# maximyudayev/Realtime-ST-GCN

Hardware: AMD Instinct MI355X
Metric: skeleton-frames/sec/GPU (fwd+bwd), 10-layer ST-GCN N=64 T=300 V=25 (higher is better)
Workload: dtype bf16; 1 GPU; config 2: as_is st-gcn (fcn_in + 9 StgcnLayer, BatchNorm, Kt=9), fwd + loss + bwd + Adam; global_batch=64, seq_len=300, joints=25, parallelism=single, bn_stats=per-replica, launch=eager

## Files before the change

realtime-st-gcn_amd/csrc/wgrad_wide.hip:

```cpp
#include "common.h"
#include "launchers.h"
#include "lds_ops.h"
#include "../../include/stgcn_amd.h"
#include <stdlib.h>

namespace {

constexpr int NT = 512;
constexpr int KM = 128;
constexpr int PR = 64;
constexpr int COB = 128, CIB = 64;
constexpr int DY_PANEL = KM * PR;
constexpr int DY_BYTES = (COB / 32) * DY_PANEL;
constexpr int DY_U = KM * (COB / 8) / NT;
constexpr int X_U = (KM * (CIB / 8) + NT - 1) / NT;
constexpr int LDS_MAX = 160 * 1024;

struct WWGeom {
  int F;
  int RS;
  int MS;
  int nco, nci;
  int tiles_n;
  int tpb;
  int R;
  int fold;
  int cin_f;
  float* slab;
};

template <int PRO, int KTAP>
__global__ __launch_bounds__(NT, 1) void wgrad_wide_kernel(const stgcn_wgrad_desc a, const WWGeom g) {
  constexpr int KT = KTAP, PADT = (KTAP - 1) / 2;
  extern __shared__ __attribute__((aligned(16))) char smem[];
  const int V = a.V, F = g.F;
  const int XP = g.MS * V * PR;
  char* const sX = smem;
  char* const sY = smem + 2 * XP;
  const int tid = threadIdx.x, lane = tid & 63, wave = tid >> 6;
  const int wc = wave >> 1, wi = wave & 1;
  {
    uint4* z = reinterpret_cast<uint4*>(smem);
    const int nz = (2 * XP + 2 * DY_BYTES) / 16;
    for (int e = tid; e < nz; e += NT) z[e] = make_uint4(0, 0, 0, 0);
    __syncthreads();
  }
  const int ob = blockIdx.x % (g.nco * g.nci), rg = blockIdx.x / (g.nco * g.nci);
  const int co0 = (ob % g.nco) * COB, cf0 = (ob / g.nco) * CIB;
  const int par = g.fold ? cf0 / a.Cin : 0;
  const int ci0 = cf0 - par * a.Cin;
  const int fmul = g.fold ? 2 : 1;
  const int tiles_n = g.tiles_n;
  const int k_begin = rg * g.tpb, k_end = min(a.N * tiles_n, k_begin + g.tpb);

  const bf16* __restrict__ xin = reinterpret_cast<const bf16*>(a.in);
  const bf16* __restrict__ dy = reinterpret_cast<const bf16*>(a.dy);

  const int ycu = tid & 15, xcu = tid & 7;
  float sc[8], sh[8];
  if (PRO == 1) {
#pragma unroll
    for (int j = 0; j < 8; ++j) {
      const int c = ci0 + xcu * 8 + j;
      sc[j] = c < a.Cin ? a.pro_a[c] : 0.f;
      sh[j] = c < a.Cin ? a.pro_b[c] : 0.f;
    }
  }
  constexpr bool AHEAD2 = KT < 9;
  uint4 ry[2][DY_U], rx[2][X_U];
  const bool ycok = co0 + ycu * 8 < a.Cout, xcok = ci0 + xcu * 8 < a.Cin;
  const bf16* __restrict__ dyb = dy + co0 + (ycok ? ycu * 8 : 0);
  const bf16* __restrict__ xb = xin + ci0 + (xcok ? xcu * 8 : 0);
  auto load_dy = [&]<int S>(int n, int f0) {
    f0 = min(f0, a.T_out - 1);
    const int rows_valid = min(F, a.T_out - f0) * V;
    const bf16* base = dyb + ((long)n * a.T_out + f0) * V * a.dy_ld;
    static_for<DY_U>([&]<int i>() {
      const int r = (tid >> 4) + 32 * i;
      ry[S][i] = *reinterpret_cast<const uint4*>(base + (long)(r < rows_valid ? r : 0) * a.dy_ld);
    });
  };
  auto store_dy = [&]<int S>(int buf, int f0) {
    const int rows_valid = ycok ? min(F, a.T_out - f0) * V : 0;
    char* p = sY + buf * DY_BYTES + (ycu >> 2) * DY_PANEL + (ycu & 3) * 16;
    static_for<DY_U>([&]<int i>() {
      const int r = (tid >> 4) + 32 * i;
      *reinterpret_cast<uint4*>(p + r * PR) = r < rows_valid ? ry[S][i] : make_uint4(0, 0, 0, 0);
    });
  };
  auto load_x = [&]<int S>(int n, int fa, int nf) {
    static_for<X_U>([&]<int i>() {
      const int r = (tid >> 3) + 64 * i;
      const int rr = r < nf * V ? r : 0;
      const int fl = rr / V, v = rr - fl * V, f = fa + fl;
      const int fs = min(max(fmul * f + par, 0), a.T_in - 1);
      rx[S][i] = *reinterpret_cast<const uint4*>(xb + (((long)n * a.T_in + fs) * V + v) * a.in_ld);
    });
  };
  auto store_x = [&]<int S>(int fa, int nf) {
    static_for<X_U>([&]<int i>() {
      const int r = (tid >> 3) + 64 * i;
      if (r < nf * V) {
        const int fl = r / V, v = r - fl * V, f = fa + fl;
        const bool ok = xcok && f >= 0 && fmul * f + par < a.T_in;
        uint4 u = ok ? rx[S][i] : make_uint4(0, 0, 0, 0);
        if (PRO == 1 && ok) {
          float e[8];
          unpack16(u, e, (bf16*)nullptr);
#pragma unroll
          for (int j = 0; j < 8; ++j) e[j] = fmaxf(fmaf(e[j], sc[j], sh[j]), 0.f);
          u = pack16(e, (bf16*)nullptr);
        }
        int slot = f % g.RS;
        slot += slot < 0 ? g.RS : 0;
        char* p = sX + (xcu >> 2) * XP + (xcu & 3) * 16 + v * PR;
        *reinterpret_cast<uint4*>(p + slot * V * PR) = u;
        if (slot + g.RS < g.MS) *reinterpret_cast<uint4*>(p + (slot + g.RS) * V * PR) = u;
      }
    });
  };
  auto stage_window = [&]<int S>(int n, int f0) {
    for (int fb = f0 - PADT; fb < f0 + F + PADT; fb += F) {
      const int nf = min(F, f0 + F + PADT - fb);
      load_x.template operator()<S>(n, fb, nf);
      store_x.template operator()<S>(fb, nf);
    }
  };

  const int li = lane & 15, gq = lane >> 4;
  const int colb = (16 * (gq & 1) + 4 * (li & 3)) * 2;
  const int rlo = 8 * (gq >> 1) + (li >> 2);

  f32x16 acc[KT];
#pragma unroll
  for (int t = 0; t < KT; ++t)
#pragma unroll
    for (int r = 0; r < 16; ++r) acc[t][r] = 0.f;

  for (int o = tid * 16; o < 2 * XP; o += NT * 16) *reinterpret_cast<uint4*>(sX + o) = make_uint4(0, 0, 0, 0);
  __syncthreads();

  const int tapb = V * PR;
  const int nk = k_end - k_begin;
  auto tile = [&]<int S>(int j) {
    const int k = k_begin + j;
    const int n = k / tiles_n, tt = k - n * tiles_n, f0 = tt * F;
    const bool next1 = j + 1 < nk && tt + 1 < tiles_n;
    if (tt == 0 || j == 0) {
      __syncthreads();
      load_dy.template operator()<S>(n, f0);
      store_dy.template operator()<S>(k & 1, f0);
      stage_window.template operator()<S>(n, f0);
      __syncthreads();
      if constexpr (AHEAD2) {
        load_dy.template operator()<S ^ 1>(n, f0 + F);
        load_x.template operator()<S ^ 1>(n, f0 + F + PADT, F);
      }
    }
    if constexpr (AHEAD2) {
      load_dy.template operator()<S>(n, f0 + 2 * F);
      load_x.template operator()<S>(n, f0 + 2 * F + PADT, F);
    } else {
      load_dy.template operator()<S ^ 1>(n, f0 + F);
      load_x.template operator()<S ^ 1>(n, f0 + F + PADT, F);
    }
    int s0 = (f0 - PADT) % g.RS;
    s0 += s0 < 0 ? g.RS : 0;
    const char* Y = sY + (k & 1) * DY_BYTES + wc * DY_PANEL + colb + rlo * PR;
    const char* X = sX + wi * XP + colb + (s0 * V + rlo) * PR;
    int tb = tapb;
    asm volatile("" : "+s"(tb));
    constexpr int NU = (KM / 16) * KT, D = 2;
    bf16x8 fx[D + 1], fy[2];
    auto rd = [&]<int u>() {
      constexpr int ks = u / KT, t = u % KT;
      if constexpr (t == 0) fy[ks & 1] = trpair<PR>(Y + 16 * ks * PR);
      fx[u % (D + 1)] = trpair<PR>(X + t * tb + 16 * ks * PR);
    };
    static_for<D>([&]<int u>() { rd.template operator()<u>(); });
    static_for<NU>([&]<int u>() {
      if constexpr (u + D < NU) rd.template operator()<u + D>();
      constexpr int ks = u / KT, t = u % KT;
      acc[t] = __builtin_amdgcn_mfma_f32_32x32x16_bf16(fy[ks & 1], fx[u % (D + 1)], acc[t], 0, 0, 0);
    });
    if (next1) {
      store_dy.template operator()<S ^ 1>((k + 1) & 1, f0 + F);
      store_x.template operator()<S ^ 1>(f0 + F + PADT, F);
    }
    lds_barrier();
  };
  for (int j = 0; j < nk; j += 2) {
    tile.template operator()<0>(j);
    if (j + 1 < nk) tile.template operator()<1>(j + 1);
  }

  float* __restrict__ out = g.slab + (long)rg * KT * a.Cout * g.cin_f;
  const int ci = cf0 + 32 * wi + (lane & 31);
#pragma unroll
  for (int t = 0; t < KT; ++t)
#pragma unroll
    for (int r = 0; r < 16; ++r) {
      const int co = co0 + 32 * wc + acc_row(r, lane);
      if (co < a.Cout && ci < g.cin_f) out[((long)t * a.Cout + co) * g.cin_f + ci] = acc[t][r];
    }
}

struct WPlan {
  bool ok;
  WWGeom g;
  int ktap;
  size_t lds;
  long slab_elems;
};

constexpr int RS_PART = 16;

__global__ void unfold_reduce2_kernel(const float* __restrict__ part, int RS, int Cout, int Cin, float* __restrict__ dw,
                                      int mode) {
  const long E4 = 5L * Cout * 2 * Cin / 4;
  const long e4 = (long)blockIdx.x * blockDim.x + threadIdx.x;
  if (e4 >= E4) return;
  const long e = e4 * 4;
  const int cf = (int)(e % (2 * Cin));
  const long tc = e / (2 * Cin);
  const int co = (int)(tc % Cout), t = (int)(tc / Cout);
  const int par = cf / Cin, ci = cf - par * Cin, dt = 2 * t + par;
  if (dt > 8) return;
  float4 acc = make_float4(0.f, 0.f, 0.f, 0.f);
  for (int r = 0; r < RS; ++r) {
    const float4 v = *reinterpret_cast<const float4*>(part + (long)r * 4 * E4 + e);
    acc.x += v.x; acc.y += v.y; acc.z += v.z; acc.w += v.w;
  }
  if (mode) {
    float* d = dw + ((long)co * Cin + ci) * 9 + dt;
    d[0] = acc.x;
    d[9] = acc.y;
    d[18] = acc.z;
    d[27] = acc.w;
    return;
  }
  float4* d = reinterpret_cast<float4*>(dw + ((long)dt * Cout + co) * Cin + ci);
  float4 o = *d;
  o.x += acc.x; o.y += acc.y; o.z += acc.z; o.w += acc.w;
  *d = o;
}

WPlan wplan(const stgcn_wgrad_desc& a) {
  WPlan p{};
  p.ok = false;
  if (a.Kt != 9 || a.pad != 4) return p;
  WWGeom& g = p.g;
  if (a.stride == 1 && a.T_in == a.T_out) {
    g.fold = 0;
    p.ktap = 9;
    g.cin_f = a.Cin;
  } else if (a.stride == 2 && a.T_out == (a.T_in - 1) / 2 + 1 && a.Cin % CIB == 0) {
    g.fold = 1;
    p.ktap = 5;
    g.cin_f = 2 * a.Cin;
  } else {
    return p;
  }
  if (a.pro != 0 && a.pro != 1) return p;
  if (a.Cout < COB || a.Cin < CIB || a.Cout % 8 || a.Cin % 8 || a.in_ld % 8 || a.dy_ld % 8 || a.V > 32) return p;
  const int padt = (p.ktap - 1) / 2;
  g.F = KM / a.V;
  g.RS = 2 * g.F + 2 * padt;
  g.MS = g.RS + g.F + 2 * padt - 1;
  if (g.F < 1 || g.F * a.V > KM || g.F * a.V > 64 * X_U) return p;
  g.nco = (a.Cout + COB - 1) / COB;
  g.nci = (g.cin_f + CIB - 1) / CIB;
  const int nob = g.nco * g.nci;
  g.tiles_n = (a.T_out + g.F - 1) / g.F;
  const long total = (long)a.N * g.tiles_n;
  if (total > 0x7fffffffL) return p;
  int R = 256 / nob;
  if (R < 1) R = 1;
  if (R > total) R = (int)total;
  g.tpb = (int)((total + R - 1) / R);
  g.R = (int)((total + g.tpb - 1) / g.tpb);
  p.lds = 2 * (size_t)g.MS * a.V * PR + 2 * (size_t)DY_BYTES;
  if (p.lds > LDS_MAX || (size_t)(KM - g.F * a.V) * PR > 2 * (size_t)DY_BYTES) return p;
  p.slab_elems = (long)(g.R + RS_PART) * p.ktap * a.Cout * g.cin_f;
  p.ok = true;
  return p;
}

}

int slab_reduce_launch(const float* slab, int R, long E, float* part, float* dw, hipStream_t s, int mode, int Kt,
                       long CoCi);
int slab_reduce1_launch(const float* slab, int R, long E, float* part, hipStream_t s);

long wgrad_wide_workspace(const stgcn_wgrad_desc& a, int dtype) {
  if (dtype != 1) return 0;
  const WPlan p = wplan(a);
  return p.ok ? p.slab_elems * (long)sizeof(float) : 0;
}

int wgrad_wide_launch(const stgcn_wgrad_desc& a, int dtype, hipStream_t s) {
  if (dtype != 1 || a.work == nullptr) return -1;
  WPlan p = wplan(a);
  if (!p.ok || a.work_bytes < p.slab_elems * (long)sizeof(float)) return -1;
  p.g.slab = reinterpret_cast<float*>(a.work);
  auto* k = p.ktap == 9 ? (a.pro == 1 ? wgrad_wide_kernel<1, 9> : wgrad_wide_kernel<0, 9>)
                        : (a.pro == 1 ? wgrad_wide_kernel<1, 5> : wgrad_wide_kernel<0, 5>);
  if (stgcn_lds_attr((const void*)k, LDS_MAX, s)) return STGCN_EHIP;
  const unsigned grid = (unsigned)(p.g.nco * p.g.nci * p.g.R);
  hipLaunchKernelGGL(k, dim3(grid), dim3(NT), p.lds, s, a, p.g);
  if (hipGetLastError() != hipSuccess) return STGCN_EHIP;
  const long E = (long)p.ktap * a.Cout * p.g.cin_f;
  float* part = p.g.slab + (long)p.g.R * E;
  if (!p.g.fold) return slab_reduce_launch(p.g.slab, p.g.R, E, part, a.dw, s, a.out_mode, 9, (long)a.Cout * a.Cin);
  const int RS = slab_reduce1_launch(p.g.slab, p.g.R, E, part, s);
  if (RS < 0) return -RS;
  hipLaunchKernelGGL(unfold_reduce2_kernel, dim3((unsigned)((E / 4 + 255) / 256)), dim3(256), 0, s, (const float*)part,
                     RS, a.Cout, a.Cin, a.dw, a.out_mode);
  return hipGetLastError() == hipSuccess ? STGCN_OK : STGCN_EHIP;
}
```

Baseline: 2.573 million skeleton-frames/s.

## Skip structurally-zero last tap in folded wgrad and batch window loads

For the folded stride-2 case with KT=5 and odd parity, the kernel now instantiates a 4-tap MFMA loop and skips the final tap, whose weight-gradient slice is presumed structurally zero, so it does no work and no writeback for it. Window staging now issues all global loads for the three frame blocks into separate register buffers before any LDS stores, which exposes more memory-level parallelism. The redundant second LDS zeroing pass and one barrier are removed, and uniform values are hinted to scalar registers. The cost is higher register pressure and a duplicated code path; the unwritten slab entries must be zero or ignored downstream for the result to stay correct.

```diff
diff --git a/realtime-st-gcn_amd/csrc/wgrad_wide.hip b/realtime-st-gcn_amd/csrc/wgrad_wide.hip
--- a/realtime-st-gcn_amd/csrc/wgrad_wide.hip
+++ b/realtime-st-gcn_amd/csrc/wgrad_wide.hip
@@ -47,7 +47,7 @@
   }
   const int ob = blockIdx.x % (g.nco * g.nci), rg = blockIdx.x / (g.nco * g.nci);
   const int co0 = (ob % g.nco) * COB, cf0 = (ob / g.nco) * CIB;
-  const int par = g.fold ? cf0 / a.Cin : 0;
+  const int par = g.fold ? __builtin_amdgcn_readfirstlane(cf0 / a.Cin) : 0;
   const int ci0 = cf0 - par * a.Cin;
   const int fmul = g.fold ? 2 : 1;
   const int tiles_n = g.tiles_n;
@@ -67,7 +67,8 @@
     }
   }
   constexpr bool AHEAD2 = KT < 9;
-  uint4 ry[2][DY_U], rx[2][X_U];
+  constexpr int NB = 3;
+  uint4 ry[2][DY_U], rx[2 + NB][X_U];
   const bool ycok = co0 + ycu * 8 < a.Cout, xcok = ci0 + xcu * 8 < a.Cin;
   const bf16* __restrict__ dyb = dy + co0 + (ycok ? ycu * 8 : 0);
   const bf16* __restrict__ xb = xin + ci0 + (xcok ? xcu * 8 : 0);
@@ -88,7 +89,7 @@
       *reinterpret_cast<uint4*>(p + r * PR) = r < rows_valid ? ry[S][i] : make_uint4(0, 0, 0, 0);
     });
   };
-  auto load_x = [&]<int S>(int n, int fa, int nf) {
+  auto load_x = [&]<int S>(int n, int fa, int nf) __attribute__((always_inline)) {
     static_for<X_U>([&]<int i>() {
       const int r = (tid >> 3) + 64 * i;
       const int rr = r < nf * V ? r : 0;
@@ -97,7 +98,7 @@
       rx[S][i] = *reinterpret_cast<const uint4*>(xb + (((long)n * a.T_in + fs) * V + v) * a.in_ld);
     });
   };
-  auto store_x = [&]<int S>(int fa, int nf) {
+  auto store_x = [&]<int S>(int fa, int nf) __attribute__((always_inline)) {
     static_for<X_U>([&]<int i>() {
       const int r = (tid >> 3) + 64 * i;
       if (r < nf * V) {
@@ -119,12 +120,11 @@
       }
     });
   };
-  auto stage_window = [&]<int S>(int n, int f0) {
-    for (int fb = f0 - PADT; fb < f0 + F + PADT; fb += F) {
-      const int nf = min(F, f0 + F + PADT - fb);
-      load_x.template operator()<S>(n, fb, nf);
-      store_x.template operator()<S>(fb, nf);
-    }
+  auto load_window = [&](int n, int f0) __attribute__((always_inline)) {
+    static_for<NB>([&]<int b>() { load_x.template operator()<2 + b>(n, f0 - PADT + b * F, min(F, F + 2 * PADT - b * F)); });
+  };
+  auto store_window = [&](int f0) __attribute__((always_inline)) {
+    static_for<NB>([&]<int b>() { store_x.template operator()<2 + b>(f0 - PADT + b * F, min(F, F + 2 * PADT - b * F)); });
   };
 
   const int li = lane & 15, gq = lane >> 4;
@@ -137,20 +137,17 @@
 #pragma unroll
     for (int r = 0; r < 16; ++r) acc[t][r] = 0.f;
 
-  for (int o = tid * 16; o < 2 * XP; o += NT * 16) *reinterpret_cast<uint4*>(sX + o) = make_uint4(0, 0, 0, 0);
-  __syncthreads();
-
   const int tapb = V * PR;
   const int nk = k_end - k_begin;
-  auto tile = [&]<int S>(int j) {
+  auto tile = [&]<int S, int NTAP>(int j) __attribute__((always_inline)) {
     const int k = k_begin + j;
     const int n = k / tiles_n, tt = k - n * tiles_n, f0 = tt * F;
     const bool next1 = j + 1 < nk && tt + 1 < tiles_n;
     if (tt == 0 || j == 0) {
-      __syncthreads();
       load_dy.template operator()<S>(n, f0);
+      load_window(n, f0);
       store_dy.template operator()<S>(k & 1, f0);
-      stage_window.template operator()<S>(n, f0);
+      store_window(f0);
       __syncthreads();
       if constexpr (AHEAD2) {
         load_dy.template operator()<S ^ 1>(n, f0 + F);
@@ -168,19 +165,19 @@
     s0 += s0 < 0 ? g.RS : 0;
     const char* Y = sY + (k & 1) * DY_BYTES + wc * DY_PANEL + colb + rlo * PR;
     const char* X = sX + wi * XP + colb + (s0 * V + rlo) * PR;
-    int tb = tapb;
+    int tb = __builtin_amdgcn_readfirstlane(tapb);
     asm volatile("" : "+s"(tb));
-    constexpr int NU = (KM / 16) * KT, D = 2;
+    constexpr int NU = (KM / 16) * NTAP, D = 2;
     bf16x8 fx[D + 1], fy[2];
     auto rd = [&]<int u>() {
-      constexpr int ks = u / KT, t = u % KT;
+      constexpr int ks = u / NTAP, t = u % NTAP;
       if constexpr (t == 0) fy[ks & 1] = trpair<PR>(Y + 16 * ks * PR);
       fx[u % (D + 1)] = trpair<PR>(X + t * tb + 16 * ks * PR);
     };
     static_for<D>([&]<int u>() { rd.template operator()<u>(); });
     static_for<NU>([&]<int u>() {
       if constexpr (u + D < NU) rd.template operator()<u + D>();
-      constexpr int ks = u / KT, t = u % KT;
+      constexpr int ks = u / NTAP, t = u % NTAP;
       acc[t] = __builtin_amdgcn_mfma_f32_32x32x16_bf16(fy[ks & 1], fx[u % (D + 1)], acc[t], 0, 0, 0);
     });
     if (next1) {
@@ -189,20 +186,31 @@
     }
     lds_barrier();
   };
-  for (int j = 0; j < nk; j += 2) {
-    tile.template operator()<0>(j);
-    if (j + 1 < nk) tile.template operator()<1>(j + 1);
+  auto run = [&]<int NTAP>() {
+    for (int j = 0; j < nk; j += 2) {
+      tile.template operator()<0, NTAP>(j);
+      if (j + 1 < nk) tile.template operator()<1, NTAP>(j + 1);
+    }
+  };
+  const bool drop_last = KT == 5 && par == 1;
+  if constexpr (KT == 5) {
+    if (drop_last) run.template operator()<KT - 1>();
+    else run.template operator()<KT>();
+  } else {
+    run.template operator()<KT>();
   }
 
   float* __restrict__ out = g.slab + (long)rg * KT * a.Cout * g.cin_f;
   const int ci = cf0 + 32 * wi + (lane & 31);
 #pragma unroll
-  for (int t = 0; t < KT; ++t)
+  for (int t = 0; t < KT; ++t) {
+    if (t == KT - 1 && drop_last) continue;
 #pragma unroll
     for (int r = 0; r < 16; ++r) {
       const int co = co0 + 32 * wc + acc_row(r, lane);
       if (co < a.Cout && ci < g.cin_f) out[((long)t * a.Cout + co) * g.cin_f + ci] = acc[t][r];
     }
+  }
 }
 
 struct WPlan {
```

Result: no change. 2.578 million skeleton-frames/s, median of 6 (+0.2%).
